# AI4Science-WestlakeU/safediffcon

Hardware: AMD Instinct MI355X
Metric: sampled control trajectories/sec (1000-step DDPM) (higher is better)
Workload: dtype f32; 1 GPU; C4: 2D smoke Unet3D_with_Conv3D dim=64 (1,2,4) state (B,32,7,64,64), B=64 per GPU, guided 1000-step DDPM, conformal quantile on; batch_per_gpu=64, global_batch=64, step=U-Net + guidance + posterior update of the whole batch, one hipGraph replay, parallelism=batch-sharded x1, no data-path collective, conv_precision=fp32

## Files before the change

include/sdc.h:

```cpp
#ifndef SDC_H
#define SDC_H

#include <stddef.h>
#include <stdint.h>

#ifdef __cplusplus
extern "C" {
#endif

#define SDC_OK 0
#define SDC_EINVAL (-1)
#define SDC_EALIGN (-2)
#define SDC_EHIP (-3)
#define SDC_ENULL (-4)

int sdc_version(void);
int sdc_last_error(char* buf, size_t cap);

typedef struct SdcConvDesc {
    int32_t B, Cin0, Cin1, Cout;
    int32_t iD, iH, iW;
    int32_t oD, oH, oW;
    int32_t kD, kH, kW;
    int32_t sD, sH, sW;
// ... 27 lines not shown

int sdc_gn_fused_ok(int B, int C, int G, int64_t S);
int sdc_gn_fused(const float* x, const float* gamma, const float* beta, const float* ss, const int32_t* t_dev,
                 int64_t ss_t_stride, int64_t ss_b_stride, int64_t ss_off, const float* residual, float* y, int B, int C, int G,
                 int64_t S, float eps, void* stream);

int sdc_gn_pointwise_out(const float* h, const float* stats, const float* gamma, const float* beta, const float* residual,
                         const float* w, const float* bias, float* y, int B, int C, int G, int Cout, int64_t S, int64_t plane,
                         int64_t ys0, int64_t ys1, int64_t ys2, void* stream);

int sdc_chan_norm(const float* x, const float* g, const float* residual, float* y, int B, int C, int64_t S,
                  int mode, float eps, void* stream);

int sdc_linattn(const float* qkv, float* ctx, float* out, int outer, int inner, int heads, int64_t n,
                int64_t q_so, int64_t q_sc, int64_t q_si, int64_t o_so, int64_t o_sc, int64_t o_si, void* stream);

size_t sdc_linattn_block_bytes(int outer, int inner, int C, int64_t n);
int sdc_linattn_block(const float* x, const float* g_pre, const float* wqkv, const float* wo, const float* bo,
                      const float* g_post, float* work, float* y, int outer, int inner, int C, int64_t n,
                      int64_t so, int64_t sc, int64_t si, int pre_mode, int post_mode, float eps, void* stream);
int sdc_linattn_block_gn(const float* x_raw, const float* gn_stats, const float* gn_gamma, const float* gn_beta, int gn_G,
                         const float* gn_residual, const float* g_pre, const float* wqkv, const float* wo, const float* bo,
                         const float* g_post, float* work, float* y, int outer, int inner, int C, int64_t n,
                         int64_t so, int64_t sc, int64_t si, int pre_mode, int post_mode, float eps, void* stream);

int sdc_tattn_block(const float* x, const float* g_pre, const float* wqkv, const float* wo, const float* rot,
                    const float* bias, float* y, int outer, int inner, int C, int ntok, int64_t so, int64_t sc,
                    int64_t st, float eps, void* stream);

size_t sdc_pack_tattn_f16_bytes(void);
int sdc_pack_tattn_f16(const float* wqkv, const float* wo, void* dst, void* stream);
int sdc_tattn_block_f16(const float* x, const float* g_pre, const void* wpk, const float* rot, const float* bias, float* y,
                        int outer, int inner, int C, int ntok, int64_t so, int64_t sc, int64_t st, float eps, void* stream);

int sdc_attn(const float* qkv, float* out, const float* rot, const float* bias, int outer, int inner, int heads,
             int ntok, int64_t q_so, int64_t q_sc, int64_t q_si, int64_t q_st,
             int64_t o_so, int64_t o_sc, int64_t o_si, int64_t o_st, void* stream);

int sdc_act(const float* x, float* y, int64_t n, int kind, void* stream);

#define SDC_MODEL_BURGERS 0
#define SDC_MODEL_TOKAMAK 1
#define SDC_MODEL_SMOKE 2

typedef struct SdcStepDesc {
    int32_t model;
    int32_t B;
    int32_t d0, d1, d2, d3;
    int32_t guide;
    int32_t clip;
    int32_t impose;
    int32_t cond_idx;
    int32_t pad_zero;
    int32_t use_max;
    int32_t has_wgt;
    int32_t skip_draws;
    int32_t ddim;
    uint64_t seed;
} SdcStepDesc;

int sdc_guide_reduce(const SdcStepDesc* d, const float* x, const float* eps, const float* coef, const int32_t* t_dev,
                     const float* gpar, float* gscal, void* stream);
int sdc_step_update(const SdcStepDesc* d, const float* x, const float* eps, const float* gext, const float* coef,
                    const int32_t* t_dev, const int32_t* draw_dev, const float* noise, int64_t noise_stride,
                    const float* gpar, const float* gscal, const float* target, const float* c0, const float* c1,
                    const float* c2, float* xout, float* x0out, void* stream);
// ... 193 lines not shown
```

safediffcon_amd/_lib.py:

```python
import ctypes as C
import os

_HERE = os.path.dirname(os.path.abspath(__file__))
LIB_PATH = os.path.join(_HERE, "libsdc_hip.so")

SDC_MODEL_BURGERS, SDC_MODEL_TOKAMAK, SDC_MODEL_SMOKE = 0, 1, 2

_f32p = C.c_void_p
_i32p = C.c_void_p
_stream = C.c_void_p
_i64 = C.c_int64


class SdcConvDesc(C.Structure):
    _fields_ = [(n, C.c_int32) for n in (
        "B", "Cin0", "Cin1", "Cout", "iD", "iH", "iW", "oD", "oH", "oW", "kD", "kH", "kW", "sD", "sH", "sW",
        "pD", "pH", "pW", "uD", "uH", "uW", "up_mode", "precision")] + [
        ("x0s", C.c_int64 * 5), ("x1s", C.c_int64 * 5), ("ys", C.c_int64 * 5), ("rs", C.c_int64 * 5)]


class SdcStepDesc(C.Structure):
    _fields_ = [(n, C.c_int32) for n in (
        "model", "B", "d0", "d1", "d2", "d3", "guide", "clip", "impose", "cond_idx", "pad_zero", "use_max",
        "has_wgt", "skip_draws", "ddim")] + [("_pad", C.c_int32), ("seed", C.c_uint64)]
# ... 37 lines not shown


SIGNATURES = {
    "sdc_version": (C.c_int, []),
    "sdc_last_error": (C.c_int, [C.c_char_p, C.c_size_t]),
    "sdc_conv": (C.c_int, [C.POINTER(SdcConvDesc), _f32p, _f32p, _f32p, _f32p, _f32p, _f32p, _stream]),
    "sdc_conv_describe": (C.c_int, [C.POINTER(SdcConvDesc), C.c_char_p, C.c_size_t, C.POINTER(C.c_double)]),
    "sdc_conv_gnparts": (C.c_int, [C.POINTER(SdcConvDesc), C.c_int]),
    "sdc_conv_gn": (C.c_int, [C.POINTER(SdcConvDesc), _f32p, _f32p, _f32p, _f32p, _f32p, _f32p, C.c_void_p, C.c_int, _stream]),
    "sdc_gn_finalize": (C.c_int, [C.c_void_p, _f32p, C.c_int, C.c_int, C.c_int, _i64, C.c_float, _stream]),
    "sdc_gn_stats": (C.c_int, [_f32p, _f32p, C.c_int, C.c_int, C.c_int, _i64, C.c_float, _stream]),
    "sdc_gn_stats_bytes": (C.c_size_t, [C.c_int, C.c_int]),
    "sdc_gn_apply": (C.c_int, [_f32p, _f32p, _f32p, _f32p, _f32p, _i32p, _i64, _i64, _i64, _f32p, _f32p,
                               C.c_int, C.c_int, C.c_int, _i64, _stream]),
    "sdc_gn_fused_ok": (C.c_int, [C.c_int, C.c_int, C.c_int, _i64]),
    "sdc_gn_fused": (C.c_int, [_f32p, _f32p, _f32p, _f32p, _i32p, _i64, _i64, _i64, _f32p, _f32p, C.c_int, C.c_int, C.c_int, _i64,
                               C.c_float, _stream]),
    "sdc_gn_pointwise_out": (C.c_int, [_f32p, _f32p, _f32p, _f32p, _f32p, _f32p, _f32p, _f32p, C.c_int, C.c_int, C.c_int, C.c_int, _i64,
                                       _i64, _i64, _i64, _i64, _stream]),
    "sdc_chan_norm": (C.c_int, [_f32p, _f32p, _f32p, _f32p, C.c_int, C.c_int, _i64, C.c_int, C.c_float, _stream]),
    "sdc_linattn": (C.c_int, [_f32p, _f32p, _f32p, C.c_int, C.c_int, C.c_int, _i64, _i64, _i64, _i64, _i64, _i64,
                              _i64, _stream]),
    "sdc_linattn_block_bytes": (C.c_size_t, [C.c_int, C.c_int, C.c_int, _i64]),
    "sdc_linattn_block": (C.c_int, [_f32p, _f32p, _f32p, _f32p, _f32p, _f32p, _f32p, _f32p, C.c_int, C.c_int, C.c_int, _i64,
                                    _i64, _i64, _i64, C.c_int, C.c_int, C.c_float, _stream]),
    "sdc_linattn_block_gn": (C.c_int, [_f32p, _f32p, _f32p, _f32p, C.c_int, _f32p, _f32p, _f32p, _f32p, _f32p, _f32p, _f32p, _f32p,
                                       C.c_int, C.c_int, C.c_int, _i64, _i64, _i64, _i64, C.c_int, C.c_int, C.c_float, _stream]),
    "sdc_tattn_block": (C.c_int, [_f32p, _f32p, _f32p, _f32p, _f32p, _f32p, _f32p, C.c_int, C.c_int, C.c_int, C.c_int,
                                  _i64, _i64, _i64, C.c_float, _stream]),
    "sdc_pack_tattn_f16_bytes": (C.c_size_t, []),
    "sdc_pack_tattn_f16": (C.c_int, [_f32p, _f32p, C.c_void_p, _stream]),
    "sdc_tattn_block_f16": (C.c_int, [_f32p, _f32p, C.c_void_p, _f32p, _f32p, _f32p, C.c_int, C.c_int, C.c_int, C.c_int,
                                      _i64, _i64, _i64, C.c_float, _stream]),
    "sdc_attn": (C.c_int, [_f32p, _f32p, _f32p, _f32p, C.c_int, C.c_int, C.c_int, C.c_int, _i64, _i64, _i64, _i64,
                           _i64, _i64, _i64, _i64, _stream]),
    "sdc_act": (C.c_int, [_f32p, _f32p, _i64, C.c_int, _stream]),
    "sdc_guide_reduce": (C.c_int, [C.POINTER(SdcStepDesc), _f32p, _f32p, _f32p, _i32p, _f32p, _f32p, _stream]),
    "sdc_step_update": (C.c_int, [C.POINTER(SdcStepDesc), _f32p, _f32p, _f32p, _f32p, _i32p, _i32p, _f32p, _i64,
                                  _f32p, _f32p, _f32p, _f32p, _f32p, _f32p, _f32p, _f32p, _stream]),
    "sdc_impose": (C.c_int, [C.POINTER(SdcStepDesc), _f32p, _f32p, _f32p, _f32p, _stream]),
    "sdc_randn": (C.c_int, [_f32p, _i64, C.c_uint64, _i32p, _stream]),
    "sdc_advance": (C.c_int, [_i32p, C.c_int, _i32p, C.c_int, _stream]),
    "sdc_advance_table": (C.c_int, [_i32p, _i32p, _i32p, _i32p, C.c_int, _stream]),
    "sdc_conformal_score": (C.c_int, [C.POINTER(SdcStepDesc), _f32p, _f32p, _f32p, _f32p, _f32p, _f32p, _stream]),
    "sdc_burgers_rollout": (C.c_int, [_f32p, _f32p, _f32p, C.c_int, C.c_int, C.c_int, C.c_int, C.c_int, C.c_float, C.c_float,
                                      C.c_float, C.c_float, C.c_float, _stream]),
    "sdc_conv_wgrad_bytes": (C.c_size_t, [C.POINTER(SdcWgradDesc)]),
    "sdc_conv_wgrad": (C.c_int, [C.POINTER(SdcWgradDesc), _f32p, _f32p, _f32p, _f32p, C.c_void_p, C.c_size_t, _stream]),
    "sdc_f16_grad_exponent": (C.c_int, [_f32p, C.c_int, C.c_int, C.c_int, C.c_int, C.c_int, C.c_void_p, C.c_void_p, _stream]),
    "sdc_conv_dgrad_f16": (C.c_int, [C.POINTER(SdcConvDesc), _f32p, _f32p, C.c_void_p, _f32p, _stream]),
    "sdc_conv_stem_f16_ok": (C.c_int, [C.POINTER(SdcConvDesc)]),
    "sdc_pack_stem_f16_bytes": (C.c_size_t, [C.c_int, C.c_int, C.c_int, C.c_int, C.c_int]),
    "sdc_pack_stem_f16": (C.c_int, [_f32p, C.c_void_p, C.c_int, C.c_int, C.c_int, C.c_int, C.c_int, _stream]),
    "sdc_conv_stem_f16": (C.c_int, [C.POINTER(SdcConvDesc), _f32p, C.c_void_p, _f32p, _f32p, _stream]),
    "sdc_conv_stem_x3_ok": (C.c_int, [C.POINTER(SdcConvDesc)]),
    "sdc_pack_stem_x3_bytes": (C.c_size_t, [C.c_int, C.c_int, C.c_int, C.c_int, C.c_int]),
    "sdc_pack_stem_x3": (C.c_int, [_f32p, C.c_void_p, C.c_int, C.c_int, C.c_int, C.c_int, C.c_int, _stream]),
    "sdc_conv_stem_x3": (C.c_int, [C.POINTER(SdcConvDesc), _f32p, C.c_void_p, _f32p, _f32p, _stream]),
    "sdc_conv_gemm_x3_ok": (C.c_int, [C.POINTER(SdcConvDesc)]),
    "sdc_pack_gemm_x3_bytes": (C.c_size_t, [C.c_int, C.c_int, C.c_int, C.c_int]),
    "sdc_pack_gemm_x3": (C.c_int, [_f32p, C.c_void_p, C.c_int, C.c_int, C.c_int, C.c_int, _stream]),
    "sdc_conv_gemm_x3": (C.c_int, [C.POINTER(SdcConvDesc), _f32p, C.c_void_p, _f32p, _f32p, _stream]),
    "sdc_conv_wino3_x3_ok": (C.c_int, [C.POINTER(SdcConvDesc)]),
    "sdc_pack_wino3_x3_bytes": (C.c_size_t, [C.c_int, C.c_int]),
    "sdc_pack_wino3_x3": (C.c_int, [_f32p, C.c_void_p, C.c_int, C.c_int, _stream]),
    "sdc_conv_wino3_x3": (C.c_int, [C.POINTER(SdcConvDesc), _f32p, _f32p, C.c_void_p, _f32p, _f32p, C.c_void_p, C.c_int, _stream]),
# ... 86 lines not shown
```

safediffcon_amd/build.py:

```python
import os
import subprocess
import sys

HERE = os.path.dirname(os.path.abspath(__file__))
CSRC = os.path.join(HERE, "csrc")
LIB = os.path.join(HERE, "libsdc_hip.so")
SOURCES = ["sdc_api.hip", "sdc_conv.hip", "sdc_conv_wino.hip", "sdc_conv_f16.hip", "sdc_conv_stem_f16.hip", "sdc_conv_stem_x3.hip", "sdc_conv_gemm_x3.hip", "sdc_conv_wino_x3.hip", "sdc_norm.hip", "sdc_attn.hip", "sdc_lablock.hip", "sdc_tablock.hip", "sdc_tablock_f16.hip", "sdc_step.hip", "sdc_solver.hip", "sdc_grad.hip", "sdc_wgrad_f16.hip", "sdc_attn_bwd.hip", "sdc_kstar.hip", "sdc_smoke.hip", "sdc_linear.hip", "sdc_optim.hip"]
HEADERS = ["sdc_common.h", "sdc_conv.h", "sdc_conv_wino3s.inc", "sdc_conv_wino2s.inc", "sdc_conv_pw2.inc"]
HIPCC = os.environ.get("HIPCC", "/opt/rocm/bin/hipcc")
FLAGS = ["--offload-arch=gfx950", "-O3", "-fPIC", "-std=c++17", "-Wall", "-Wno-unused-function"]


def source_hash():
    import hashlib
    h = hashlib.sha256()
    for f in SOURCES + HEADERS:
        with open(os.path.join(CSRC, f), "rb") as fh:
            h.update(fh.read())
    with open(os.path.join(HERE, "..", "include", "sdc.h"), "rb") as fh:
        h.update(fh.read())
    return h.hexdigest()[:16]


def _stale(out, deps):
    if not os.path.exists(out):
        return True
    t = os.path.getmtime(out)
    return any(os.path.getmtime(d) > t for d in deps)


def build_experiments(verbose=True):
    out = os.path.join(HERE, "libsdc_hip_exp.so")
    cmd = [HIPCC, *FLAGS, "-DSDC_KERNEL_EXPERIMENTS", "-shared", *[os.path.join(CSRC, s) for s in SOURCES], "-o", out]
    if verbose:
        print(" ".join(cmd), flush=True)
    subprocess.check_call(cmd)
    return out


def build(force=False, verbose=True, jobs=4):
# ... 28 lines not shown
```

safediffcon_amd/engine.py:

```python
import ctypes as C
import functools
import os
import math

import torch

from . import _lib
from ._lib import SdcConvDesc, check


def _ptr(t):
    return 0 if t is None else t.data_ptr()


def _s5(t):
    assert t.dim() == 5, t.shape
    return tuple(int(s) for s in t.stride())


def as5(t):
    while t.dim() < 5:
        t = t.unsqueeze(2)
    return t

# ... 77 lines not shown
def pack_stem_f16(w):
    t5 = as5(w).to(torch.float32)
    co, ci, kD, kH, kW = t5.shape
    if not (kW == 7 and (kD, kH) in ((1, 1), (1, 7), (7, 7)) and 1 <= ci <= 8):
        raise ValueError(f"pack_stem_f16: taps 1x1x7, 1x7x7 or 7x7x7 and Cin <= 8 (got {tuple(t5.shape)})")
    taps, ns = kH * 7, (kH * 7 + 1) // 2
    z = t5.new_zeros(co, 8, kD, 2 * ns)
    z[:, :ci, :, :taps] = t5.reshape(co, ci, kD, taps)
    z = z.reshape(co, 8, kD, ns, 2).permute(2, 3, 0, 4, 1).contiguous()
    return z.half().reshape(-1).view(torch.float32)


def pack_stem_x3(w):
    t5 = as5(w).to(torch.float32)
    co, ci, kD, kH, kW = t5.shape
    if not (kW == 7 and (kD, kH) in ((1, 1), (1, 7), (7, 7)) and 1 <= ci <= 8):
        raise ValueError(f"pack_stem_x3: taps 1x1x7, 1x7x7 or 7x7x7 and Cin <= 8 (got {tuple(t5.shape)})")
    taps, ns = kH * 7, (kH * 7 + 1) // 2
    z = t5.new_zeros(co, 8, kD, 2 * ns)
    z[:, :ci, :, :taps] = t5.reshape(co, ci, kD, taps)
    z = z.reshape(co, 8, kD, ns, 2).permute(2, 3, 0, 4, 1).contiguous()
    return torch.stack(split3_bf16(z)).reshape(-1).view(torch.float32)


def pack_tattn_f16(wqkv, wo):
    wqkv, wo = wqkv.to(torch.float32), wo.to(torch.float32)
    if tuple(wqkv.shape) != (384, 64) or tuple(wo.shape) != (64, 128):
        raise ValueError(f"pack_tattn_f16: to_qkv (384, 64) and to_out (64, 128) (got {tuple(wqkv.shape)}, {tuple(wo.shape)})")
    a = wqkv.reshape(3, 4, 32, 4, 2, 8).permute(1, 0, 3, 4, 2, 5)
    b = wo.reshape(2, 32, 4, 2, 2, 2, 4).permute(2, 0, 3, 5, 1, 4, 6)
    return torch.cat([a.reshape(-1), b.reshape(-1)]).half().view(torch.float32)


def pack_gemm_x3(wp, cout, cin, k):
    k = tuple(k)[-2:]
    ncb = {(4, 4): 1, (2, 2): 2, (1, 1): 4}.get(k, 0)
    taps = k[0] * k[1]
    if ncb == 0 or cout <= 0 or cout % 64 or cin <= 0 or cin % (16 * ncb) or tuple(wp.shape) != (taps * cin, cout):
        raise ValueError(f"pack_gemm_x3: taps 4x4, 2x2 or 1x1, Cout % 64 == 0, Cin % {16 * max(ncb, 1)} == 0, Wp [taps * Cin][Cout] "
                         f"(got taps {k}, Cin {cin}, Cout {cout}, Wp {tuple(wp.shape)})")
    z = wp.to(torch.float32).reshape(taps, cin // (16 * ncb), ncb, 16, cout // 64, 64)
    z = z.permute(4, 1, 2, 0, 5, 3).contiguous()
    return torch.stack(split3_bf16(z)).reshape(-1).view(torch.float32)


def pack_wino3_x3(wp4, cout, cin):
    n = 64 * cin * cout
    if cout <= 0 or cout % 64 or cin <= 0 or cin % 16 or wp4.dim() != 1 or wp4.numel() != (27 + 36 + 48 + 64) * cin * cout:
        raise ValueError(f"pack_wino3_x3: Cout % 64 == 0, Cin % 16 == 0, the flat precision-4 buffer of a 3x3x3 conv "
                         f"(got Cin {cin}, Cout {cout}, {tuple(wp4.shape)})")
    u3 = wp4[-n:].to(torch.float32).reshape(4, cin // 16, 16, cout // 64, 64, 4, 4)
    z = u3.permute(3, 0, 1, 5, 6, 4, 2).reshape(cout // 64, 4, cin // 16, 4, 4, 4, 2, 8, 2, 8)
    z = torch.stack((z[:, :, :, :, :, :, 0], z[:, :, :, :, :, :, 1].flip(-2)), 6).contiguous()
    return torch.stack(split3_bf16(z)).reshape(-1).view(torch.float32)


def split3_bf16(x):
    h = x.bfloat16()
    r = x - h.float()
    m = r.bfloat16()
    return h, m, (r - m.float()).bfloat16()


def conv_precision(n, k, cin, cout, f16=None, train=False):
    floats = functools.partial(_lib.get_lib().sdc_pack_conv_weight_floats, cout, cin, *k)
    if train:
# ... 17 lines not shown
    d.uD, d.uH, d.uW = up
    d.up_mode, d.precision = up_mode, precision
    d.x0s[:] = _s5(x)
    d.x1s[:] = _s5(x1) if x1 is not None else (0,) * 5
    d.ys[:] = _s5(out)
    d.rs[:] = _s5(residual) if residual is not None else (0,) * 5
    return d


class Pool:

    def __init__(self, device):
        self.device = device
        self.free = {}
        self.all = []
        self.bytes = 0

    def get(self, shape):
        n = int(math.prod(shape))
        lst = self.free.get(n)
        if lst:
            return lst.pop().view(shape)
        t = torch.empty(n, dtype=torch.float32, device=self.device)
        self.all.append(t)
        self.bytes += n * 4
        return t.view(shape)

    def put(self, t):
        self.free.setdefault(t.numel(), []).append(t.reshape(-1))


class Plan:

    def __init__(self, device, precision=0, stem_f16=False, stem_split=False, gemm_split=False, attn_f16=False, wino_split=False):
        self.device = torch.device(device)
        self.lib = _lib.get_lib()
        self.precision = int(precision)
        if self.precision not in (0, 2, 3, 4, 5, 6, 7):
            raise ValueError(f"precision must be 0, 2, 3, 4, 5, 6 or 7 (got {precision})")
        self.stem_f16 = bool(stem_f16)
        self.stem_split = bool(stem_split) and self.precision >= 4 and not self.stem_f16
        self.gemm_split = bool(gemm_split) and self.precision >= 4
        self.wino_split = bool(wino_split) and self.precision in (4, 5)
        self.attn_f16 = bool(attn_f16)
        self.calls = []
        self.pool = Pool(self.device)
        self.keep = []
        self.repackers = []
        self._stats = None
        self._ctx = None
        self._gn_parts = {}
        self.fuse_gn_stats = True
        self.fuse_gn_small = True
        self.split_small_grids = False

    def run(self, stream):
        for fn, args in self.calls:
            rc = fn(*args, stream)
            if rc:
                check(rc, fn.__name__)

    def refresh_weights(self):
        with torch.no_grad():
            for dst, fn in self.repackers:
                dst.copy_(fn())

    def _stats_buf(self, B, G):
        need = int(self.lib.sdc_gn_stats_bytes(B, G))
        if self._stats is None or self._stats.numel() * 4 < need:
            self._stats = torch.empty((need + 3) // 4, dtype=torch.float32, device=self.device)
            self.keep.append(self._stats)
        return self._stats

    def _ctx_buf(self, n):
        if self._ctx is None or self._ctx.numel() < n:
            self._ctx = torch.empty(n, dtype=torch.float32, device=self.device)
            self.keep.append(self._ctx)
# ... 179 lines not shown
        st, gamma, beta, groups, res = gn
        B, Cc = x.shape[0], x.shape[1]
        S = x.numel() // (B * Cc)
        cout = out.shape[1]
        plane = out.shape[3] * out.shape[4]
        ys = _s5(out)
        ok = (x.is_contiguous() and (res is None or res.is_contiguous()) and cout <= 16 and Cc % 4 == 0 and Cc <= 2048 and S >= 1024 and plane % 4 == 0 and ys[4] == 1 and
              ys[3] == out.shape[4] and all(v % 4 == 0 for v in ys[:3]) and out.data_ptr() % 16 == 0 and
              tuple(out.shape[2:]) == tuple(x.shape[2:]))
        if not ok:
            return None
        self.keep += [x, st, gamma, beta, res, w, bias, out]
        self._emit(self.lib.sdc_gn_pointwise_out, _ptr(x), _ptr(st), _ptr(gamma), _ptr(beta), _ptr(res), _ptr(w), _ptr(bias), _ptr(out),
                   B, Cc, groups, cout, S, plane, ys[0], ys[1], ys[2])
        return out

    def linattn_block(self, x, g_pre, wqkv, wo, bo, g_post, outer, inner, n, strides, pre_mode, post_mode, eps=1e-5, gn=None):
        Cc = x.shape[1]
        y = self.pool.get(tuple(x.shape))
        work = torch.empty(int(self.lib.sdc_linattn_block_bytes(outer, inner, Cc, n)) // 4, dtype=torch.float32, device=self.device)
        self.keep += [x, g_pre, wqkv, wo, bo, g_post, work, y]
        if gn is not None:
            st, gamma, beta, groups, res = gn
            assert outer == x.shape[0] and (res is None or (tuple(res.shape) == tuple(x.shape) and res.stride() == x.stride()))
            self.keep += [st, gamma, beta, res]
            self._emit(self.lib.sdc_linattn_block_gn, _ptr(x), _ptr(st), _ptr(gamma), _ptr(beta), groups, _ptr(res), _ptr(g_pre),
                       _ptr(wqkv), _ptr(wo), _ptr(bo), _ptr(g_post), _ptr(work), _ptr(y), outer, inner, Cc, n, *strides, pre_mode,
                       post_mode, eps)
            return y
        self._emit(self.lib.sdc_linattn_block, _ptr(x), _ptr(g_pre), _ptr(wqkv), _ptr(wo), _ptr(bo), _ptr(g_post), _ptr(work),
                   _ptr(y), outer, inner, Cc, n, *strides, pre_mode, post_mode, eps)
        return y

    def tattn_weight(self, wqkv, wo):
        return self.packed(lambda: pack_tattn_f16(wqkv() if callable(wqkv) else wqkv, wo() if callable(wo) else wo))

    def tattn_block(self, x, g_pre, wqkv, wo, rot, bias, eps=1e-5):
        B, Cc, Fr, H, W = x.shape
        assert x.is_contiguous()
        y = self.pool.get(tuple(x.shape))
        if self.attn_f16:
            wpk = self.tattn_weight(wqkv, wo)
            self.keep += [x, g_pre, wpk, rot, bias, y]
            self._emit(self.lib.sdc_tattn_block_f16, _ptr(x), _ptr(g_pre), _ptr(wpk), _ptr(rot), _ptr(bias), _ptr(y),
                       B, H * W, Cc, Fr, Cc * Fr * H * W, Fr * H * W, H * W, eps)
            return y
        self.keep += [x, g_pre, wqkv, wo, rot, bias, y]
        self._emit(self.lib.sdc_tattn_block, _ptr(x), _ptr(g_pre), _ptr(wqkv), _ptr(wo), _ptr(rot), _ptr(bias), _ptr(y),
                   B, H * W, Cc, Fr, Cc * Fr * H * W, Fr * H * W, H * W, eps)
        return y

    def attn(self, qkv, out, heads, outer, inner, ntok, q_strides, o_strides, rot=None, bias=None):
        self.keep += [qkv, out, rot, bias]
        self._emit(self.lib.sdc_attn, _ptr(qkv), _ptr(out), _ptr(rot), _ptr(bias), outer, inner, heads, ntok,
                   *q_strides, *o_strides)
        return out
```

safediffcon_amd/unet.py:

```python
import ctypes as C
import functools
import math
import os

import torch
from torch import nn

from ._lib import check, get_lib
from .engine import Plan, as5, pack_conv_weight

HEADS, DIM_HEAD = 4, 32
HID = HEADS * DIM_HEAD


def _resnet_spec(p, cin, cout, time_dim, k):
    s = []
    if time_dim is not None:
        s += [(f"{p}.mlp.1.weight", (cout * 2, time_dim)), (f"{p}.mlp.1.bias", (cout * 2,))]
    for blk, ci in (("block1", cin), ("block2", cout)):
        s += [(f"{p}.{blk}.proj.weight", (cout, ci, *k)), (f"{p}.{blk}.proj.bias", (cout,)),
              (f"{p}.{blk}.norm.weight", (cout,)), (f"{p}.{blk}.norm.bias", (cout,))]
    if cin != cout:
        s += [(f"{p}.res_conv.weight", (cout, cin, *([1] * len(k)))), (f"{p}.res_conv.bias", (cout,))]
    return s
# ... 220 lines not shown
        pool.put(h)
        own = net.has(f"{prefix}.res_conv.weight")
        if own:
            r = self.conv(x, f"{prefix}.res_conv", x1=x1)
        else:
            assert x1 is None
            r = x
        if defer_gn:
            st = self.plan.gn_stats_deferred(g, groups)
            return g, (st, self.V(f"{prefix}.block2.norm.weight"), self.V(f"{prefix}.block2.norm.bias"), groups, r), (r if own else None)
        self.gn(g, f"{prefix}.block2.norm", groups, residual=r)
        if own:
            pool.put(r)
        return g


class _HipUNet(nn.Module):

    def __init__(self, spec, dim, seed=None):
        super().__init__()
        gen = torch.Generator()
        gen.manual_seed(int(torch.initial_seed()) & 0x7FFFFFFF if seed is None else seed)
        for k, v in _default_init(spec, gen).items():
            _register(self, k, v)
        self._spec = spec
        self._plans = {}
        self.precision = 4
        self.train_precision = None
        self.stem_f16 = False
        self.attn_f16 = False
        self.stem_split = True
        self.gemm_split = True
        self.wino_split = True
        self.fuse_linattn = True
        self.fuse_gn_into_linattn = True
        self.content_stamp = True
        self.subpixel_upsample = True
        self.split_small_grids = False
        self.fuse_final_conv = True
        self.forward_graph = True
        self._side = None
        self.dim = dim
        self.self_condition = False
        self.cond_offsets, off = {}, 0
        for k, shape in spec:
            if k.endswith(".mlp.1.weight"):
                self.cond_offsets[k[: -len(".mlp.1.weight")]] = off
                off += shape[0]
        self.cond_width = off

    @property
    def train_precision(self):
        return self.__dict__.get("_train_precision")

    @train_precision.setter
    def train_precision(self, v):
        from .autograd import check_train_precision
        self.__dict__["_train_precision"] = check_train_precision(v)

    def P(self, key):
        m = self
        *mods, leaf = key.split(".")
        for name in mods:
            m = m._modules[name]
        return m._parameters[leaf]

# ... 56 lines not shown
            tab = self._span_tab = (key, host.to(dev), torch.zeros(1, dtype=torch.int64, device=dev))
        lib = get_lib()
        check(lib.sdc_checksum_spans(tab[1].data_ptr(), len(ts), tab[2].data_ptr(), torch.cuda.current_stream(dev).cuda_stream),
              "sdc_checksum_spans")
        return int(tab[2].item())

    def _weights_stamp(self):
        host = hash(tuple((p.data_ptr(), p._version) for p in self.parameters()))
        dev = next(self.parameters()).device
        if not (self.content_stamp and dev.type == "cuda"):
            return (host, 0)
        if torch.cuda.is_current_stream_capturing():
            return (host, getattr(self, "_last_content", 0))
        self._last_content = self._content_stamp()
        return (host, self._last_content)

    def _refresh_entry(self, e, stamp):
        e["plan"].refresh_weights()
        e["cond"].refresh_weights()
        e["lut_valid"] = False
        e["wstamp"] = stamp

    def refresh(self):
        stamp = self._weights_stamp()
        for e in self._plans.values():
            self._refresh_entry(e, stamp)

    def device(self):
        return next(self.parameters()).device

    def entry(self, shape, rows, lut=False):
        key = (tuple(shape), rows, bool(lut), int(self.precision), bool(self.fuse_linattn), bool(self.subpixel_upsample),
               bool(self.fuse_gn_into_linattn), bool(self.split_small_grids), bool(self.fuse_final_conv), bool(self.stem_f16),
               bool(self.stem_split), bool(self.gemm_split), bool(self.attn_f16), bool(self.wino_split))
        stamp = self._weights_stamp()
        ent = self._plans.get(key)
        if ent is not None and ent["wstamp"] != stamp:
            self._refresh_entry(ent, stamp)
        if key not in self._plans:
            dev = self.device()
            if dev.type != "cuda":
                raise RuntimeError("safediffcon_amd runs on MI355X only: move the model to a cuda (HIP) device; "
                                   "there is no CPU fallback")
            plan = Plan(dev, precision=self.precision, stem_f16=bool(self.stem_f16), stem_split=bool(self.stem_split),
                        gemm_split=bool(self.gemm_split), attn_f16=bool(self.attn_f16), wino_split=bool(self.wino_split))
            plan.split_small_grids = bool(self.split_small_grids)
            x = torch.zeros(shape, dtype=torch.float32, device=dev)
            eps = torch.zeros(shape, dtype=torch.float32, device=dev)
            b = _Builder(self, plan)
            self._build(b, x, eps)
            plan.cond_sites = b.cond_sites
            cond = Plan(dev)
            td = self.dim * 4
            emb = torch.zeros((rows, self.dim, 1, 1, 1), dtype=torch.float32, device=dev)
            cb = _Builder(self, cond)
            h = cb.conv(emb, "time_mlp.1")
            cond.act(h, 1)
            temb = cb.conv(h, "time_mlp.3")
            cond.act(temb, 0)
            prefixes = list(self.cond_offsets)
            wcat = cond.conv_weight(lambda: torch.cat([self.P(f"{p}.mlp.1.weight") for p in prefixes], 0))
            bcat = cond.vec(lambda: torch.cat([self.P(f"{p}.mlp.1.bias") for p in prefixes], 0))
            ss = cond.conv(temb, wcat, bcat, self.cond_width, (1, 1, 1))
            assert temb.shape[1] == td
            self._plans[key] = dict(plan=plan, cond=cond, x=x, eps=eps, emb=emb, ss=ss, rows=rows, lut_valid=False,
                                    t_dev=None, wstamp=stamp)
        return self._plans[key]

    def bind_cond(self, ent, t_dev):
        plan, ss, W = ent["plan"], ent["ss"], self.cond_width
        for idx, off in plan.cond_sites:
            fn, a = plan.calls[idx]
            a = list(a)
            i0 = 3 if fn is plan.lib.sdc_gn_fused else 4
            if t_dev is None:
                a[i0:i0 + 5] = ss.data_ptr(), 0, 0, W, off
            else:
                a[i0:i0 + 5] = ss.data_ptr(), t_dev.data_ptr(), W, 0, off
# ... 192 lines not shown
        if (cond_dim is not None or out_dim is not None or use_bert_text_cond or init_dim is not None
                or init_kernel_size != 7 or not use_sparse_linear_attn or attn_heads != 4 or attn_dim_head != 32):
            raise NotImplementedError("options never enabled by the reference's 2D scripts are not built")
        super().__init__(spec_smoke(dim, tuple(dim_mults), channels), dim)
        self.channels, self.dim_mults, self.groups = channels, tuple(dim_mults), resnet_groups
        self.has_cond = False
        shared = self.P("init_temporal_attn.fn.fn.fn.rotary_emb.freqs")
        shared.requires_grad_(False)
        for k, _ in self._spec:
            if k.endswith("rotary_emb.freqs"):
                m = self
                for name in k.split(".")[:-1]:
                    m = m._modules[name]
                m._parameters["freqs"] = shared

    def _attn_tables(self, b, F):
        plan = b.plan
        if not hasattr(plan, "_rot"):
            def rot():
                fr = self.P("init_temporal_attn.fn.fn.fn.rotary_emb.freqs").detach().float().cpu()
                ang = torch.arange(F, dtype=torch.float32)[:, None] * fr[None, :]
                return torch.stack((ang.cos(), ang.sin()), dim=-1).reshape(-1)
            plan._rot = plan.packed(rot)
            plan._bias = plan.packed(lambda: rel_pos_bias_table(
                self.P("time_rel_pos_bias.relative_attention_bias.weight").detach(), F).reshape(-1))
        return plan._rot, plan._bias

    def _temporal(self, b, prefix, x):
        plan, pool = b.plan, b.plan.pool
        B, C, F, H, W = x.shape
        hw = H * W
        rot, bias = self._attn_tables(b, F)
        if self.fuse_linattn and C == 64 and F == 32 and hw % 8 == 0 and x.is_contiguous():
            if plan.attn_f16:
                return plan.tattn_block(x, b.V(f"{prefix}.fn.norm.gamma"), lambda: self.P(f"{prefix}.fn.fn.fn.to_qkv.weight"),
                                        lambda: self.P(f"{prefix}.fn.fn.fn.to_out.weight"), rot, bias)
            return plan.tattn_block(x, b.V(f"{prefix}.fn.norm.gamma"), b.W(f"{prefix}.fn.fn.fn.to_qkv.weight"),
                                    b.W(f"{prefix}.fn.fn.fn.to_out.weight"), rot, bias)
        xn = plan.chan_norm(x, b.V(f"{prefix}.fn.norm.gamma"), 0)
        qkv = b.conv(xn, f"{prefix}.fn.fn.fn.to_qkv", bias=False)
        pool.put(xn)
        o = pool.get((B, HID, F, H, W))
        plan.attn(qkv, o, HEADS, B, hw, F, (3 * HID * F * hw, F * hw, 1, hw), (HID * F * hw, F * hw, 1, hw), rot, bias)
        pool.put(qkv)
        y = b.conv(o, f"{prefix}.fn.fn.fn.to_out", bias=False, residual=x)
        pool.put(o)
        return y

    def _la_fusable(self, shape):
        B, C, F, H, W = shape
        return self.fuse_linattn and C in (64, 128) and (H * W) % 64 == 0 and B * F < 65536

    def _resnet_then_spatial_linear(self, b, res_prefix, la_prefix, x, G):
        pool = b.plan.pool
        cout = self.P(f"{res_prefix}.block2.proj.weight").shape[0]
        if self.fuse_gn_into_linattn and self._la_fusable((x.shape[0], cout, *x.shape[2:])):
            g, gn, r = b.resnet(res_prefix, x, G, defer_gn=True)
            y = self._spatial_linear(b, la_prefix, g, gn=gn)
            if r is not None:
                pool.put(r)
            return y, g
        a = b.resnet(res_prefix, x, G)
        return self._spatial_linear(b, la_prefix, a), a

    def _spatial_linear(self, b, prefix, x, gn=None):
        plan, pool = b.plan, b.plan.pool
        B, C, F, H, W = x.shape
# ... 79 lines not shown
```

Baseline: 0.2970 trajectories/s.

## Add bf16x3-split MFMA temporal attention block kernel for 64ch/32-frame case

Adds a fused temporal-attention kernel that splits fp32 activations and weights into three bf16 parts and runs the QKV and output projections on bf16 MFMA with six partial products, emulating fp32 accuracy. Weights are pre-packed per head and double-buffered in LDS while the next head is fetched. It is routed only when precision is 4/5, attn_f16 is off, and the shape is C=64, 32 frames, 4096 pixels, replacing the fp32 fused tattn block. The cost is extra MFMA work for the splits and a large LDS footprint, with accuracy close to but not identical with fp32.

```diff
diff --git a/include/sdc.h b/include/sdc.h
--- a/include/sdc.h
+++ b/include/sdc.h
@@ -83,6 +83,12 @@
 int sdc_pack_tattn_f16(const float* wqkv, const float* wo, void* dst, void* stream);
 int sdc_tattn_block_f16(const float* x, const float* g_pre, const void* wpk, const float* rot, const float* bias, float* y,
                         int outer, int inner, int C, int ntok, int64_t so, int64_t sc, int64_t st, float eps, void* stream);
+
+size_t sdc_pack_tattn_x3_bytes(void);
+int sdc_pack_tattn_x3(const float* wqkv, const float* wo, void* dst, void* stream);
+int sdc_tattn_block_x3(const float* x, const float* g_pre, const void* wpk, const float* rot, const float* bias, float* y,
+                       int outer, int inner, int C, int ntok, int64_t so, int64_t sc, int64_t st, float eps, void* stream);
+int sdc_tattn_block_x3_ok(int C, int ntok, int inner);
 
 int sdc_attn(const float* qkv, float* out, const float* rot, const float* bias, int outer, int inner, int heads,
              int ntok, int64_t q_so, int64_t q_sc, int64_t q_si, int64_t q_st,
diff --git a/safediffcon_amd/_lib.py b/safediffcon_amd/_lib.py
--- a/safediffcon_amd/_lib.py
+++ b/safediffcon_amd/_lib.py
@@ -93,6 +93,11 @@
     "sdc_pack_tattn_f16": (C.c_int, [_f32p, _f32p, C.c_void_p, _stream]),
     "sdc_tattn_block_f16": (C.c_int, [_f32p, _f32p, C.c_void_p, _f32p, _f32p, _f32p, C.c_int, C.c_int, C.c_int, C.c_int,
                                       _i64, _i64, _i64, C.c_float, _stream]),
+    "sdc_pack_tattn_x3_bytes": (C.c_size_t, []),
+    "sdc_pack_tattn_x3": (C.c_int, [_f32p, _f32p, C.c_void_p, _stream]),
+    "sdc_tattn_block_x3": (C.c_int, [_f32p, _f32p, C.c_void_p, _f32p, _f32p, _f32p, C.c_int, C.c_int, C.c_int, C.c_int,
+                                     _i64, _i64, _i64, C.c_float, _stream]),
+    "sdc_tattn_block_x3_ok": (C.c_int, [C.c_int, C.c_int, C.c_int]),
     "sdc_attn": (C.c_int, [_f32p, _f32p, _f32p, _f32p, C.c_int, C.c_int, C.c_int, C.c_int, _i64, _i64, _i64, _i64,
                            _i64, _i64, _i64, _i64, _stream]),
     "sdc_act": (C.c_int, [_f32p, _f32p, _i64, C.c_int, _stream]),
diff --git a/safediffcon_amd/build.py b/safediffcon_amd/build.py
--- a/safediffcon_amd/build.py
+++ b/safediffcon_amd/build.py
@@ -5,7 +5,7 @@
 HERE = os.path.dirname(os.path.abspath(__file__))
 CSRC = os.path.join(HERE, "csrc")
 LIB = os.path.join(HERE, "libsdc_hip.so")
-SOURCES = ["sdc_api.hip", "sdc_conv.hip", "sdc_conv_wino.hip", "sdc_conv_f16.hip", "sdc_conv_stem_f16.hip", "sdc_conv_stem_x3.hip", "sdc_conv_gemm_x3.hip", "sdc_conv_wino_x3.hip", "sdc_norm.hip", "sdc_attn.hip", "sdc_lablock.hip", "sdc_tablock.hip", "sdc_tablock_f16.hip", "sdc_step.hip", "sdc_solver.hip", "sdc_grad.hip", "sdc_wgrad_f16.hip", "sdc_attn_bwd.hip", "sdc_kstar.hip", "sdc_smoke.hip", "sdc_linear.hip", "sdc_optim.hip"]
+SOURCES = ["sdc_api.hip", "sdc_conv.hip", "sdc_conv_wino.hip", "sdc_conv_f16.hip", "sdc_conv_stem_f16.hip", "sdc_conv_stem_x3.hip", "sdc_conv_gemm_x3.hip", "sdc_conv_wino_x3.hip", "sdc_norm.hip", "sdc_attn.hip", "sdc_lablock.hip", "sdc_tablock.hip", "sdc_tablock_f16.hip", "sdc_tablock_x3.hip", "sdc_step.hip", "sdc_solver.hip", "sdc_grad.hip", "sdc_wgrad_f16.hip", "sdc_attn_bwd.hip", "sdc_kstar.hip", "sdc_smoke.hip", "sdc_linear.hip", "sdc_optim.hip"]
 HEADERS = ["sdc_common.h", "sdc_conv.h", "sdc_conv_wino3s.inc", "sdc_conv_wino2s.inc", "sdc_conv_pw2.inc"]
 HIPCC = os.environ.get("HIPCC", "/opt/rocm/bin/hipcc")
 FLAGS = ["--offload-arch=gfx950", "-O3", "-fPIC", "-std=c++17", "-Wall", "-Wno-unused-function"]
diff --git a/safediffcon_amd/csrc/sdc_tablock_x3.hip b/safediffcon_amd/csrc/sdc_tablock_x3.hip
--- /dev/null
+++ b/safediffcon_amd/csrc/sdc_tablock_x3.hip
@@ -0,0 +1,328 @@
+#include "sdc_common.h"
+
+namespace {
+
+constexpr int NT = 512;
+constexpr int C = 64;
+constexpr int NS = 8;
+constexpr int XP = NS * 33;
+constexpr int XF = 68;
+constexpr int XPP = 32 * XF + 8;
+constexpr int WQKV_E = 3 * 4 * 64 * 8;
+constexpr int HEAD_E = WQKV_E + 2 * 2 * 64 * 8;
+constexpr int WPK_E = 4 * 3 * HEAD_E;
+constexpr int WBUF_B = 3 * HEAD_E * 2;
+constexpr int REGB_B = NS * XPP * 4;
+typedef float f32x16 __attribute__((ext_vector_type(16)));
+typedef float nfloat4 __attribute__((ext_vector_type(4)));
+typedef __bf16 bf16x8 __attribute__((ext_vector_type(8)));
+typedef uint32_t u32x4 __attribute__((ext_vector_type(4)));
+static_assert(WBUF_B <= REGB_B && 32 * XP * 4 <= REGB_B, "region B holds a head's weights and a y half");
+static_assert(WBUF_B % (16 * NT) == 0, "whole 16-byte words per thread");
+
+struct TaArgs {
+    const float* x; const float* g; const __bf16* wpk; const float* rot; const float* bias;
+    float* y;
+    int inner;
+    int nblk;
+    float eps;
+    int64_t so, sc, st;
+};
+
+__host__ __device__ __forceinline__ int crow(int r, int lh) { return (r & 3) + 8 * (r >> 2) + 4 * lh; }
+
+typedef __attribute__((address_space(1))) float* gptr_t;
+typedef __attribute__((address_space(1))) char* gcptr_t;
+__device__ __forceinline__ gptr_t uni(const float* p) {
+    const uint64_t u = reinterpret_cast<uint64_t>(p);
+    const uint32_t lo = __builtin_amdgcn_readfirstlane((uint32_t)u), hi = __builtin_amdgcn_readfirstlane((uint32_t)(u >> 32));
+    return (gptr_t)(((uint64_t)hi << 32) | lo);
+}
+__device__ __forceinline__ float ldu(gptr_t base, uint32_t byte_off) { return *(gptr_t)((gcptr_t)base + byte_off); }
+__device__ __forceinline__ void stu(gptr_t base, uint32_t byte_off, float v) { *(gptr_t)((gcptr_t)base + byte_off) = v; }
+
+typedef float ta2 __attribute__((ext_vector_type(2)));
+__device__ __forceinline__ ta2 ta_rot(ta2 x, ta2 cs) {
+#pragma clang fp contract(off)
+    const float t0 = x.x * cs.x, t1 = x.y * cs.x;
+    return ta2{__builtin_fmaf(-x.y, cs.y, t0), __builtin_fmaf(x.x, cs.y, t1)};
+}
+
+__device__ __forceinline__ void split3(float x, __bf16& h, __bf16& m, __bf16& l) {
+#pragma clang fp contract(off)
+    h = (__bf16)x;
+    const float r = x - (float)h;
+    m = (__bf16)r;
+    l = (__bf16)(r - (float)m);
+}
+
+__global__ __launch_bounds__(NT) void ta_block_x3_kernel(const TaArgs a) {
+    extern __shared__ __attribute__((aligned(16))) unsigned char smem_x3[];
+    unsigned char* const wA = smem_x3;
+    unsigned char* const rB = smem_x3 + WBUF_B;
+    float* const xim = reinterpret_cast<float*>(rB);
+    float* const ys = reinterpret_cast<float*>(rB);
+    float* const biasT = reinterpret_cast<float*>(rB + REGB_B);
+    float* const rotcs = biasT + 4 * 32 * 33;
+    float* const red = rotcs + 2 * 32 * 16;
+
+    const int tid = threadIdx.x, lane = tid & 63, wave = tid >> 6, l31 = lane & 31, lh = lane >> 5;
+    const int nblk = a.nblk, nwg = gridDim.x, w = blockIdx.x;
+    const bool xcd = ((nblk & 7) == 0) && ((nwg & 7) == 0);
+    const int per = xcd ? (nblk >> 3) : nblk;
+    const int base = xcd ? (w & 7) * per : 0;
+    const int first = xcd ? (w >> 3) : w, stride = xcd ? (nwg >> 3) : nwg;
+
+    const int tok = tid & 255, half = tid >> 8, pw = tok & 7, f = tok >> 3;
+    const uint32_t toff = (uint32_t)(((int64_t)f * a.st + pw) * 4);
+    auto tile_ptr = [&](int li) -> int64_t {
+        const int seq0 = (base + li) * NS;
+        const int o = seq0 / a.inner, i0 = seq0 - o * a.inner;
+        return (int64_t)o * a.so + i0;
+    };
+
+    u32x4 wreg[6];
+    auto fetch_head = [&](int head) {
+        const u32x4* src = reinterpret_cast<const u32x4*>(a.wpk) + head * (WBUF_B / 16) + tid;
+#pragma unroll
+        for (int i = 0; i < 6; ++i) wreg[i] = src[i * NT];
+    };
+    auto park_head = [&](unsigned char* wb) {
+        u32x4* dst = reinterpret_cast<u32x4*>(wb) + tid;
+#pragma unroll
+        for (int i = 0; i < 6; ++i) dst[i * NT] = wreg[i];
+    };
+
+    float v[32];
+    if (first < per) {
+        const float* xt = a.x + tile_ptr(first) + (int64_t)(half * 32) * a.sc;
+#pragma unroll
+        for (int c = 0; c < 32; ++c) v[c] = ldu(uni(xt + (int64_t)c * a.sc), toff);
+    }
+    {
+        fetch_head(0);
+#pragma unroll
+        for (int i = 0; i < 8; ++i) {
+            const int e = tid + i * NT, h = e >> 10, q = (e >> 5) & 31, kk = e & 31;
+            biasT[(h * 32 + kk) * 33 + q] = (a.bias ? a.bias[e] : 0.0f) * 5.65685424949238f;
+        }
+        const float2 rr = a.rot ? *reinterpret_cast<const float2*>(a.rot + tid * 2) : make_float2(1.0f, 0.0f);
+        *reinterpret_cast<float2*>(rotcs + (((tid & 15) * 32) + (tid >> 4)) * 2) = rr;
+        park_head(wA);
+    }
+    const int hw = wave;
+
+    for (int li = first; li < per; li += stride) {
+        const int64_t tp = tile_ptr(li);
+        const bool more = li + stride < per;
+        {
+            float sm = 0.f;
+#pragma unroll
+            for (int c = 0; c < 32; ++c) sm += v[c];
+            red[half * 256 + tok] = sm;
+            __syncthreads();
+            const float mean = (red[tok] + red[256 + tok]) * (1.0f / C);
+            float q = 0.f;
+#pragma unroll
+            for (int c = 0; c < 32; ++c) { v[c] -= mean; q += v[c] * v[c]; }
+            red[512 + half * 256 + tok] = q;
+            __syncthreads();
+            const float rstd = rsqrtf((red[512 + tok] + red[768 + tok]) * (1.0f / C) + a.eps);
+            nfloat4* xo = reinterpret_cast<nfloat4*>(xim + pw * XPP + f * XF + half * 32);
+#pragma unroll
+            for (int c4 = 0; c4 < 8; ++c4) {
+                nfloat4 o;
+#pragma unroll
+                for (int j = 0; j < 4; ++j) o[j] = v[c4 * 4 + j] * rstd * a.g[half * 32 + c4 * 4 + j];
+                xo[c4] = o;
+            }
+        }
+        __syncthreads();
+        bf16x8 xf[3][4];
+        {
+            const float* xr = xim + hw * XPP + l31 * XF + 8 * lh;
+#pragma unroll
+            for (int s = 0; s < 4; ++s) {
+                const nfloat4 lo = *reinterpret_cast<const nfloat4*>(xr + 16 * s), hi = *reinterpret_cast<const nfloat4*>(xr + 16 * s + 4);
+#pragma unroll
+                for (int j = 0; j < 8; ++j) {
+                    __bf16 ph, pm, pl;
+                    split3(j < 4 ? lo[j] : hi[j - 4], ph, pm, pl);
+                    xf[0][s][j] = ph; xf[1][s][j] = pm; xf[2][s][j] = pl;
+                }
+            }
+        }
+        f32x16 yacc[2];
+#pragma unroll
+        for (int i = 0; i < 2; ++i)
+#pragma unroll
+            for (int r = 0; r < 16; ++r) yacc[i][r] = 0.f;
+#pragma unroll 1
+        for (int head = 0; head < 4; ++head) {
+            constexpr int PA[6] = {2, 1, 0, 1, 0, 0}, PB[6] = {0, 1, 2, 0, 1, 0};
+            const unsigned char* const wh = (head & 1) ? rB : wA;
+            unsigned char* const wn = (head & 1) ? wA : rB;
+            __syncthreads();
+            const bool next = head < 3 || more;
+            if (next) fetch_head((head + 1) & 3);
+            const bf16x8* wf = reinterpret_cast<const bf16x8*>(wh) + lane;
+            f32x16 q, k, vt;
+#pragma unroll
+            for (int r = 0; r < 16; ++r) { q[r] = 0.f; k[r] = 0.f; vt[r] = 0.f; }
+#pragma unroll
+            for (int t = 0; t < 6; ++t)
+#pragma unroll
+                for (int s = 0; s < 4; ++s) {
+                    const bf16x8* wp = wf + PA[t] * (HEAD_E / 8);
+                    q = __builtin_amdgcn_mfma_f32_32x32x16_bf16(wp[(0 * 4 + s) * 64], xf[PB[t]][s], q, 0, 0, 0);
+                    k = __builtin_amdgcn_mfma_f32_32x32x16_bf16(wp[(1 * 4 + s) * 64], xf[PB[t]][s], k, 0, 0, 0);
+                    vt = __builtin_amdgcn_mfma_f32_32x32x16_bf16(xf[PB[t]][s], wp[(2 * 4 + s) * 64], vt, 0, 0, 0);
+                    if (s == 3) __builtin_amdgcn_sched_barrier(0);
+                }
+            if (next) park_head(wn);
+#pragma unroll
+            for (int r = 0; r < 16; r += 2) {
+                const int m = crow(r, lh) >> 1;
+                const ta2 cs = *reinterpret_cast<const ta2*>(rotcs + (m * 32 + l31) * 2);
+                ta2 q2 = {q[r], q[r + 1]}, k2 = {k[r], k[r + 1]};
+                q2 = ta_rot(q2, cs);
+                k2 = ta_rot(k2, cs);
+                q[r] = q2.x; q[r + 1] = q2.y;
+                k[r] = k2.x; k[r + 1] = k2.y;
+            }
+            f32x16 acc;
+#pragma unroll
+            for (int r = 0; r < 16; ++r) acc[r] = biasT[(head * 32 + crow(r, lh)) * 33 + l31];
+#pragma unroll
+            for (int r = 0; r < 16; ++r) acc = __builtin_amdgcn_mfma_f32_32x32x2f32(k[r], q[r], acc, 0, 0, 0);
+            float mx = -INFINITY;
+#pragma unroll
+            for (int r = 0; r < 16; ++r) mx = fmaxf(mx, acc[r]);
+            mx = fmaxf(mx, __shfl_xor(mx, 32, 64));
+            const float SL = 0.17677669529663687f * 1.4426950408889634f;
+            const float nmx = -mx * SL;
+            float sum = 0.f;
+#pragma unroll
+            for (int r = 0; r < 16; ++r) { acc[r] = __builtin_amdgcn_exp2f(fmaf(acc[r], SL, nmx)); sum += acc[r]; }
+            sum += __shfl_xor(sum, 32, 64);
+            const float inv = 1.0f / sum;
+#pragma unroll
+            for (int r = 0; r < 16; ++r) acc[r] *= inv;
+            f32x16 oacc;
+#pragma unroll
+            for (int r = 0; r < 16; ++r) oacc[r] = 0.f;
+#pragma unroll
+            for (int r = 0; r < 16; ++r) oacc = __builtin_amdgcn_mfma_f32_32x32x2f32(vt[r], acc[r], oacc, 0, 0, 0);
+            bf16x8 of[3][2];
+#pragma unroll
+            for (int s = 0; s < 2; ++s)
+#pragma unroll
+                for (int j = 0; j < 8; ++j) {
+                    __bf16 ph, pm, pl;
+                    split3(oacc[8 * s + j], ph, pm, pl);
+                    of[0][s][j] = ph; of[1][s][j] = pm; of[2][s][j] = pl;
+                }
+            const bf16x8* wof = wf + WQKV_E / 8;
+#pragma unroll
+            for (int t = 0; t < 6; ++t)
+#pragma unroll
+                for (int s = 0; s < 2; ++s) {
+                    const bf16x8* wp = wof + PA[t] * (HEAD_E / 8);
+                    yacc[0] = __builtin_amdgcn_mfma_f32_32x32x16_bf16(wp[(0 * 2 + s) * 64], of[PB[t]][s], yacc[0], 0, 0, 0);
+                    yacc[1] = __builtin_amdgcn_mfma_f32_32x32x16_bf16(wp[(1 * 2 + s) * 64], of[PB[t]][s], yacc[1], 0, 0, 0);
+                }
+        }
+        {
+            const float* xt = a.x + tile_ptr(more ? li + stride : li) + (int64_t)(half * 32) * a.sc;
+#pragma unroll
+            for (int c = 0; c < 32; ++c) v[c] = ldu(uni(xt + (int64_t)c * a.sc), toff);
+        }
+#pragma unroll
+        for (int i = 0; i < 2; ++i) {
+            float xr[16];
+            const int64_t ch0 = (int64_t)(i * 32 + half * 16) * a.sc;
+            const float* xt = a.x + tp + ch0;
+#pragma unroll
+            for (int c = 0; c < 16; ++c) xr[c] = ldu(uni(xt + (int64_t)c * a.sc), toff);
+            __syncthreads();
+#pragma unroll
+            for (int r = 0; r < 16; ++r) ys[crow(r, lh) * XP + hw * 33 + l31] = yacc[i][r];
+            __syncthreads();
+            const float* yt = a.y + tp + ch0;
+#pragma unroll
+            for (int c = 0; c < 16; ++c) stu(uni(yt + (int64_t)c * a.sc), toff, ys[(half * 16 + c) * XP + pw * 33 + f] + xr[c]);
+        }
+        __syncthreads();
+    }
+}
+
+__global__ __launch_bounds__(256) void pack_tattn_x3_kernel(const float* __restrict__ wqkv, const float* __restrict__ wo,
+                                                            __bf16* __restrict__ dst) {
+    const int g = blockIdx.x * 256 + threadIdx.x;
+    if (g >= 4 * HEAD_E) return;
+    const int head = g / HEAD_E, e = g - head * HEAD_E;
+    const int j = e & 7, lane = (e >> 3) & 63, l31 = lane & 31, lh = lane >> 5;
+    float wv;
+    if (e < WQKV_E) {
+        const int s = (e >> 9) & 3, mat = e >> 11;
+        wv = wqkv[(mat * 128 + head * 32 + l31) * C + 16 * s + 8 * lh + j];
+    } else {
+        const int e2 = e - WQKV_E, s = (e2 >> 9) & 1, i = (e2 >> 10) & 1;
+        wv = wo[(32 * i + l31) * 128 + head * 32 + crow(8 * s + j, lh)];
+    }
+    __bf16 ph, pm, pl;
+    split3(wv, ph, pm, pl);
+    __bf16* d = dst + (int64_t)head * 3 * HEAD_E + e;
+    d[0] = ph; d[HEAD_E] = pm; d[2 * HEAD_E] = pl;
+}
+
+bool sdc_tattn_x3_faster(int Cc, int ntok, int inner) {
+    return Cc == 64 && ntok == 32 && inner == 4096;
+}
+
+}
+
+extern "C" int sdc_tattn_block_x3_ok(int Cc, int ntok, int inner) { return sdc_tattn_x3_faster(Cc, ntok, inner) ? 1 : 0; }
+
+extern "C" size_t sdc_pack_tattn_x3_bytes(void) { return (size_t)WPK_E * sizeof(__bf16); }
+
+extern "C" int sdc_pack_tattn_x3(const float* wqkv, const float* wo, void* dst, void* stream) {
+    SDC_REQUIRE(wqkv && wo && dst, SDC_ENULL, "sdc_pack_tattn_x3: null pointer");
+    SDC_REQUIRE(reinterpret_cast<uintptr_t>(dst) % 16 == 0, SDC_EALIGN, "sdc_pack_tattn_x3: dst must be 16-byte aligned");
+    hipLaunchKernelGGL(pack_tattn_x3_kernel, dim3(4 * HEAD_E / 256), dim3(256), 0, sdc::as_stream(stream), wqkv, wo,
+                       reinterpret_cast<__bf16*>(dst));
+    return sdc::check_launch("sdc_pack_tattn_x3");
+}
+
+extern "C" int sdc_tattn_block_x3(const float* x, const float* g_pre, const void* wpk, const float* rot, const float* bias, float* y,
+                                  int outer, int inner, int Cc, int ntok, int64_t so, int64_t sc, int64_t st, float eps, void* stream) {
+    SDC_REQUIRE(x && g_pre && wpk && y, SDC_ENULL, "sdc_tattn_block_x3: null pointer");
+    SDC_REQUIRE(Cc == 64 && ntok == 32, SDC_EINVAL, "sdc_tattn_block_x3: dim 64 and 32 frames only (got %d, %d)", Cc, ntok);
+    SDC_REQUIRE(outer > 0 && inner > 0 && inner % NS == 0, SDC_EINVAL, "sdc_tattn_block_x3: pixels per image must be a multiple of 8");
+    const int64_t nblk = (int64_t)outer * inner / NS;
+    SDC_REQUIRE(nblk < (1ll << 31), SDC_EINVAL, "sdc_tattn_block_x3: too many sequences");
+    SDC_REQUIRE(((int64_t)31 * st + inner + (int64_t)63 * sc) * 4 < (1ll << 32) && so >= 0 && sc >= 0 && st >= 0, SDC_EINVAL,
+                "sdc_tattn_block_x3: one outer index must span less than 4 GB (32-bit lane offsets)");
+    SDC_REQUIRE(reinterpret_cast<uintptr_t>(wpk) % 16 == 0, SDC_EALIGN, "sdc_tattn_block_x3: the weight buffer must be 16-byte aligned");
+    SDC_REQUIRE(!rot || reinterpret_cast<uintptr_t>(rot) % 8 == 0, SDC_EINVAL, "sdc_tattn_block_x3: rot must be 8-byte aligned");
+    TaArgs a;
+    a.x = x; a.g = g_pre; a.wpk = reinterpret_cast<const __bf16*>(wpk); a.rot = rot; a.bias = bias; a.y = y;
+    a.inner = inner; a.nblk = (int)nblk; a.eps = eps; a.so = so; a.sc = sc; a.st = st;
+    const size_t ldsb = (size_t)WBUF_B + REGB_B + sizeof(float) * (size_t)(4 * 32 * 33 + 2 * 32 * 16 + 1024);
+    static std::atomic<uint64_t> attr{0};
+    SDC_LDS_OPTIN(attr, ta_block_x3_kernel, 160 * 1024, "sdc_tattn_block_x3");
+    static std::atomic<int> ncu_of[64];
+    int dev = 0;
+    if (hipGetDevice(&dev) != hipSuccess || dev < 0 || dev >= 64) { sdc::set_error("sdc_tattn_block_x3: hipGetDevice failed"); return SDC_EHIP; }
+    int ncu = ncu_of[dev].load(std::memory_order_acquire);
+    if (ncu <= 0) {
+        if (hipDeviceGetAttribute(&ncu, hipDeviceAttributeMultiprocessorCount, dev) != hipSuccess || ncu <= 0) {
+            sdc::set_error("sdc_tattn_block_x3: cannot read the CU count of device %d", dev);
+            return SDC_EHIP;
+        }
+        ncu_of[dev].store(ncu, std::memory_order_release);
+    }
+    const unsigned grid = (unsigned)(nblk < ncu ? nblk : ncu);
+    hipLaunchKernelGGL(ta_block_x3_kernel, dim3(grid), dim3(NT), ldsb, sdc::as_stream(stream), a);
+    return sdc::check_launch("sdc_tattn_block_x3");
+}
diff --git a/safediffcon_amd/engine.py b/safediffcon_amd/engine.py
--- a/safediffcon_amd/engine.py
+++ b/safediffcon_amd/engine.py
@@ -133,6 +133,16 @@
     return torch.cat([a.reshape(-1), b.reshape(-1)]).half().view(torch.float32)
 
 
+def pack_tattn_x3(wqkv, wo):
+    wqkv, wo = wqkv.to(torch.float32), wo.to(torch.float32)
+    if tuple(wqkv.shape) != (384, 64) or tuple(wo.shape) != (64, 128):
+        raise ValueError(f"pack_tattn_x3: to_qkv (384, 64) and to_out (64, 128) (got {tuple(wqkv.shape)}, {tuple(wo.shape)})")
+    a = wqkv.reshape(3, 4, 32, 4, 2, 8).permute(1, 0, 3, 4, 2, 5)
+    b = wo.reshape(2, 32, 4, 2, 2, 2, 4).permute(2, 0, 3, 5, 1, 4, 6)
+    z = torch.cat([a.reshape(4, -1), b.reshape(4, -1)], 1)
+    return torch.stack(split3_bf16(z), 1).reshape(-1).view(torch.float32)
+
+
 def pack_gemm_x3(wp, cout, cin, k):
     k = tuple(k)[-2:]
     ncb = {(4, 4): 1, (2, 2): 2, (1, 1): 4}.get(k, 0)
@@ -216,7 +226,8 @@
 
 class Plan:
 
-    def __init__(self, device, precision=0, stem_f16=False, stem_split=False, gemm_split=False, attn_f16=False, wino_split=False):
+    def __init__(self, device, precision=0, stem_f16=False, stem_split=False, gemm_split=False, attn_f16=False, wino_split=False,
+                 attn_split=False):
         self.device = torch.device(device)
         self.lib = _lib.get_lib()
         self.precision = int(precision)
@@ -227,6 +238,7 @@
         self.gemm_split = bool(gemm_split) and self.precision >= 4
         self.wino_split = bool(wino_split) and self.precision in (4, 5)
         self.attn_f16 = bool(attn_f16)
+        self.attn_split = bool(attn_split) and self.precision in (4, 5) and not self.attn_f16
         self.calls = []
         self.pool = Pool(self.device)
         self.keep = []
@@ -472,13 +484,23 @@
                    _ptr(y), outer, inner, Cc, n, *strides, pre_mode, post_mode, eps)
         return y
 
-    def tattn_weight(self, wqkv, wo):
-        return self.packed(lambda: pack_tattn_f16(wqkv() if callable(wqkv) else wqkv, wo() if callable(wo) else wo))
+    def tattn_weight(self, wqkv, wo, split=False):
+        pack = pack_tattn_x3 if split else pack_tattn_f16
+        return self.packed(lambda: pack(wqkv() if callable(wqkv) else wqkv, wo() if callable(wo) else wo))
+
+    def tattn_split_routes(self, Cc, Fr, hw):
+        return self.attn_split and bool(self.lib.sdc_tattn_block_x3_ok(int(Cc), int(Fr), int(hw)))
 
     def tattn_block(self, x, g_pre, wqkv, wo, rot, bias, eps=1e-5):
         B, Cc, Fr, H, W = x.shape
         assert x.is_contiguous()
         y = self.pool.get(tuple(x.shape))
+        if self.tattn_split_routes(Cc, Fr, H * W):
+            wpk = self.tattn_weight(wqkv, wo, split=True)
+            self.keep += [x, g_pre, wpk, rot, bias, y]
+            self._emit(self.lib.sdc_tattn_block_x3, _ptr(x), _ptr(g_pre), _ptr(wpk), _ptr(rot), _ptr(bias), _ptr(y),
+                       B, H * W, Cc, Fr, Cc * Fr * H * W, Fr * H * W, H * W, eps)
+            return y
         if self.attn_f16:
             wpk = self.tattn_weight(wqkv, wo)
             self.keep += [x, g_pre, wpk, rot, bias, y]
diff --git a/safediffcon_amd/unet.py b/safediffcon_amd/unet.py
--- a/safediffcon_amd/unet.py
+++ b/safediffcon_amd/unet.py
@@ -276,6 +276,7 @@
         self.stem_split = True
         self.gemm_split = True
         self.wino_split = True
+        self.attn_split = True
         self.fuse_linattn = True
         self.fuse_gn_into_linattn = True
         self.content_stamp = True
@@ -398,7 +399,7 @@
     def entry(self, shape, rows, lut=False):
         key = (tuple(shape), rows, bool(lut), int(self.precision), bool(self.fuse_linattn), bool(self.subpixel_upsample),
                bool(self.fuse_gn_into_linattn), bool(self.split_small_grids), bool(self.fuse_final_conv), bool(self.stem_f16),
-               bool(self.stem_split), bool(self.gemm_split), bool(self.attn_f16), bool(self.wino_split))
+               bool(self.stem_split), bool(self.gemm_split), bool(self.attn_f16), bool(self.wino_split), bool(self.attn_split))
         stamp = self._weights_stamp()
         ent = self._plans.get(key)
         if ent is not None and ent["wstamp"] != stamp:
@@ -409,7 +410,8 @@
                 raise RuntimeError("safediffcon_amd runs on MI355X only: move the model to a cuda (HIP) device; "
                                    "there is no CPU fallback")
             plan = Plan(dev, precision=self.precision, stem_f16=bool(self.stem_f16), stem_split=bool(self.stem_split),
-                        gemm_split=bool(self.gemm_split), attn_f16=bool(self.attn_f16), wino_split=bool(self.wino_split))
+                        gemm_split=bool(self.gemm_split), attn_f16=bool(self.attn_f16), wino_split=bool(self.wino_split),
+                        attn_split=bool(self.attn_split))
             plan.split_small_grids = bool(self.split_small_grids)
             x = torch.zeros(shape, dtype=torch.float32, device=dev)
             eps = torch.zeros(shape, dtype=torch.float32, device=dev)
@@ -668,7 +670,7 @@
         hw = H * W
         rot, bias = self._attn_tables(b, F)
         if self.fuse_linattn and C == 64 and F == 32 and hw % 8 == 0 and x.is_contiguous():
-            if plan.attn_f16:
+            if plan.attn_f16 or plan.tattn_split_routes(C, F, hw):
                 return plan.tattn_block(x, b.V(f"{prefix}.fn.norm.gamma"), lambda: self.P(f"{prefix}.fn.fn.fn.to_qkv.weight"),
                                         lambda: self.P(f"{prefix}.fn.fn.fn.to_out.weight"), rot, bias)
             return plan.tattn_block(x, b.V(f"{prefix}.fn.norm.gamma"), b.W(f"{prefix}.fn.fn.fn.to_qkv.weight"),
```

Result: faster. 0.3036 trajectories/s (median of 6 runs) (+2.2%).
